# G1OJS/PyFT8

Hardware: NVIDIA B200
Metric: decoded 15-s FT8 cycles/sec (higher is better)
Workload: dtype f32

## Files before the change

pyft8_b200/csrc/fine_tc.cuh:

```cuda
#pragma once
#include <cuda_runtime.h>
#include <stdint.h>
#include "fine.cuh"

namespace ft8 {

struct TScanOut { int32_t tt; float score0; };

constexpr int FS_WIN = 224;
constexpr int FS_CAND = 32;
constexpr int FS_K1 = 64, FS_NU = 328, FS_K = FS_K1 + FS_NU, FS_KC = 8, FS_CHUNKS = FS_K / FS_KC;
constexpr int FS_N = 64;
constexpr int FS_TILES = 4;
constexpr int FS_STAGES = 4;
constexpr int FS_ACC_COLS = FS_TILES * FS_N;
constexpr int FS_A_STAGE_COLS = FS_TILES * 16;
constexpr int FS_B_SPLIT_BYTES = 2 * FS_N * 16;
constexpr int FS_B_STAGE_BYTES = 2 * FS_B_SPLIT_BYTES;
constexpr int FS_GEN_WARPS = 16;
constexpr int FS_BSTAGES = 8;
constexpr int FS_ISSUERS = 4;
constexpr int FS_NT = (FS_GEN_WARPS + FS_ISSUERS + 1) * 32;
constexpr int FS_W_LEN = 6400;
constexpr int FS_SMEM_BYTES = FS_BSTAGES * FS_B_STAGE_BYTES + FS_W_LEN * 8;
constexpr int FS_BMAT_FLOATS = FS_CHUNKS * FS_B_STAGE_BYTES / 4;
static_assert(FS_ACC_COLS + FS_STAGES * FS_A_STAGE_COLS == 512, "TMEM column plan");

__host__ __device__ __forceinline__ int fs_u_of(int j) { return j < 164 ? j - 182 : j + 554; }

__device__ __forceinline__ uint32_t smem_u32(const void* p) { return (uint32_t)__cvta_generic_to_shared(p); }
__device__ __forceinline__ void mbar_init(uint32_t a, int count) { asm volatile("mbarrier.init.shared::cta.b64 [%0], %1;" ::"r"(a), "r"(count)); }
__device__ __forceinline__ void mbar_expect_tx(uint32_t a, int bytes) {
    asm volatile("mbarrier.arrive.expect_tx.shared::cta.b64 _, [%0], %1;" ::"r"(a), "r"(bytes) : "memory");
}
__device__ __forceinline__ void mbar_wait(uint32_t a, uint32_t parity) {
    uint32_t done = 0;
    for (uint32_t spin = 0; !done; ++spin) {
        asm volatile("{\n\t.reg .pred p;\n\tmbarrier.try_wait.parity.shared::cta.b64 p, [%1], %2;\n\tselp.u32 %0, 1, 0, p;\n\t}"
                     : "=r"(done) : "r"(a), "r"(parity) : "memory");
        if (spin > (1u << 24)) __trap();
    }
}
__device__ __forceinline__ void bulk_g2s(uint32_t dst, const void* src, int bytes, uint32_t mbar) {
    asm volatile("cp.async.bulk.shared::cluster.global.mbarrier::complete_tx::bytes [%0], [%1], %2, [%3];"
                 ::"r"(dst), "l"(src), "r"(bytes), "r"(mbar) : "memory");
}
__device__ __forceinline__ void fence_proxy_async() { asm volatile("fence.proxy.async.shared::cta;" ::: "memory"); }
__device__ __forceinline__ void tc_fence_before() { asm volatile("tcgen05.fence::before_thread_sync;" ::: "memory"); }
__device__ __forceinline__ void tc_fence_after() { asm volatile("tcgen05.fence::after_thread_sync;" ::: "memory"); }
__device__ __forceinline__ void tc_commit(uint32_t mbar) {
    asm volatile("tcgen05.commit.cta_group::1.mbarrier::arrive::one.shared::cluster.b64 [%0];" ::"r"(mbar) : "memory");
}
__device__ __forceinline__ uint64_t umma_desc(uint32_t saddr, int lbo_bytes, int sbo_bytes) {
    return (uint64_t)((saddr >> 4) & 0x3FFF) | ((uint64_t)((lbo_bytes >> 4) & 0x3FFF) << 16) | ((uint64_t)((sbo_bytes >> 4) & 0x3FFF) << 32) |
           (1ull << 46);
}
constexpr uint32_t FS_IDESC = (1u << 4) | (2u << 7) | (2u << 10) | ((FS_N >> 3) << 17) | ((128u >> 4) << 24);
__device__ __forceinline__ void umma_tf32(uint32_t d_tmem, uint64_t da, uint64_t db, uint32_t accumulate) {
    asm volatile("{\n\t.reg .pred p;\n\tsetp.ne.b32 p, %4, 0;\n\t"
                 "tcgen05.mma.cta_group::1.kind::tf32 [%0], %1, %2, %3, {%5, %5, %5, %5}, p;\n\t}"
                 ::"r"(d_tmem), "l"(da), "l"(db), "r"(FS_IDESC), "r"(accumulate), "r"(0u) : "memory");
}
__device__ __forceinline__ void tmem_ld32(uint32_t taddr, uint32_t (&v)[32]) {
    asm volatile("tcgen05.ld.sync.aligned.32x32b.x32.b32 "
                 "{%0, %1, %2, %3, %4, %5, %6, %7, %8, %9, %10, %11, %12, %13, %14, %15, "
                 "%16, %17, %18, %19, %20, %21, %22, %23, %24, %25, %26, %27, %28, %29, %30, %31}, [%32];"
                 : "=r"(v[0]), "=r"(v[1]), "=r"(v[2]), "=r"(v[3]), "=r"(v[4]), "=r"(v[5]), "=r"(v[6]), "=r"(v[7]), "=r"(v[8]), "=r"(v[9]),
                   "=r"(v[10]), "=r"(v[11]), "=r"(v[12]), "=r"(v[13]), "=r"(v[14]), "=r"(v[15]), "=r"(v[16]), "=r"(v[17]), "=r"(v[18]),
                   "=r"(v[19]), "=r"(v[20]), "=r"(v[21]), "=r"(v[22]), "=r"(v[23]), "=r"(v[24]), "=r"(v[25]), "=r"(v[26]), "=r"(v[27]),
                   "=r"(v[28]), "=r"(v[29]), "=r"(v[30]), "=r"(v[31])
                 : "r"(taddr) : "memory");
}
__device__ __forceinline__ void tmem_ld_wait() { asm volatile("tcgen05.wait::ld.sync.aligned;" ::: "memory"); }
__device__ __forceinline__ float4 ldg_v4_pinned(const void* p) {
    float4 v;
    asm volatile("ld.global.nc.v4.f32 {%0, %1, %2, %3}, [%4];" : "=f"(v.x), "=f"(v.y), "=f"(v.z), "=f"(v.w) : "l"(p));
    return v;
}
__device__ __forceinline__ float2 ldg_v2_pinned(const void* p) {
    float2 v;
    asm volatile("ld.global.nc.v2.f32 {%0, %1}, [%2];" : "=f"(v.x), "=f"(v.y) : "l"(p));
    return v;
}
__device__ __forceinline__ float tf32_hi(float x) { return __uint_as_float(__float_as_uint(x) & 0xFFFFE000u); }

__device__ __forceinline__ void fine_pass12_split_finish(const FineIn& in, float2* dst, int tid, const float2* __restrict__ TF,
                                                         const float* taper, const float2 (&w)[8]) {
    const int p2 = tid & 127;
    float2 ax[4] = {in.ax[0], in.ax[1], in.ax[2], in.ax[3]};
    if (p2 >= 110) ax[0] = cscale(taper[p2 - 110], ax[0]);
    if (p2 < 82) ax[1] = cscale(taper[p2 + 18], ax[1]);
    if (p2 >= 106) ax[2] = cscale(taper[p2 - 106], ax[2]);
    if (p2 < 78) ax[3] = cscale(taper[p2 + 22], ax[3]);
    if (tid < 128) {
        fine_pass12_col<0>(in, ax, dst, p2, TF, w);
        fine_pass12_col<1>(in, ax, dst, p2, TF, w);
        fine_pass12_col<2>(in, ax, dst, p2, TF, w);
    } else {
        fine_pass12_col<3>(in, ax, dst, p2, TF, w);
        fine_pass12_col<4>(in, ax, dst, p2, TF, w);
    }
}

template <int NT>
__device__ __forceinline__ void fine_pass3_nt(const float2* src, float2* dst, int tid, const float2 (&tw8)[7]) {
    const int p = tid & 15;
#pragma unroll
    for (int r = 0; r < (25 * 16 + NT - 1) / NT; ++r) {
        const int q = (tid >> 4) + (NT / 16) * r;
        if (q < 25) {
            float2 a[8];
#pragma unroll
            for (int j = 0; j < 8; ++j) a[j] = src[q + 25 * p + 400 * j];
            Dft<8, true>::run(a);
            float2* d = dst + q + 201 * p;
            d[0] = a[0];
#pragma unroll
            for (int k = 1; k < 8; ++k) d[25 * k] = cmulc(a[k], tw8[k - 1]);
        }
    }
    __syncthreads();
}

template <int NT>
__device__ __forceinline__ void fine_last_full_nt(const float2* src, float2* dst, int tid) {
#pragma unroll
    for (int t0 = 0; t0 < 200; t0 += NT) {
        const int t = t0 + tid;
        if (t < 200) {
            float2 a[16];
#pragma unroll
            for (int j = 0; j < 16; ++j) a[j] = src[t + 201 * j];
            Dft<16, true>::run(a);
#pragma unroll
            for (int k = 0; k < 16; ++k) dst[t + 200 * k] = a[k];
        }
    }
    __syncthreads();
}

template <int NT>
__device__ __forceinline__ void fine_pass12_finish_nt(const FineIn& in, float2* dst, int tid, const float2* __restrict__ TF,
                                                      const float* taper, const float2 (&w)[8]) {
    if (NT == 256) fine_pass12_split_finish(in, dst, tid, TF, taper, w);
    else fine_pass12_finish(in, dst, tid, TF, taper, w);
}

struct FineItem { int slot, f0, h0, cyc, tt, ff; };

#ifndef FT_NT
#define FT_NT 128
#endif
#ifndef FT_CTAS
#define FT_CTAS (FT_NT == 128 ? 4 : 2)
#endif
#ifndef FF_CTAS
#define FF_CTAS (FT_NT == 128 ? 3 : 2)
#endif
constexpr int FT_SMEM_BYTES = (FINE_N + FINE_NP) * (int)sizeof(float2) + (16 + 100) * (int)sizeof(float) + (32 + 16 + 256) * (int)sizeof(float2);

template <int NT, int CTAS>
__global__ void __launch_bounds__(NT, CTAS)
k_fine_tscan(const float2* __restrict__ spec, int spec_stride, const int32_t* __restrict__ list, const int32_t* __restrict__ count,
             int n_direct, const int32_t* __restrict__ cycle_of, const int16_t* __restrict__ cand_f0, const int16_t* __restrict__ cand_h0,
             const float2* __restrict__ TF, TScanOut* __restrict__ tso, float2* __restrict__ zwin_out) {
    extern __shared__ float2 fine_smem[];
    float2 *px = fine_smem, *po = fine_smem + FINE_N;
    float* score = reinterpret_cast<float*>(fine_smem + FINE_N + FINE_NP);
    float* taper = score + 16;
    float2* w32 = reinterpret_cast<float2*>(taper + 100);
    float2* w16 = w32 + 32;
    float2* zwin = w16 + 16;
    const int tid = threadIdx.x, lane = tid & 31, warp = tid >> 5;
    if (tid < 32) w32[tid] = c_fine.w32[tid];
    if (tid < 16) { const float2 w = c_fine.w32[2 * tid]; w16[tid] = make_float2(w.x, -w.y); }
    if (tid < 100) taper[tid] = c_fine.taper[tid];
    __syncthreads();
    float2 tw[8];
#pragma unroll
    for (int t = 0; t < 8; ++t) tw[t] = w32[(t * (lane & 7)) & 31];
    float2 tw5[8];
#pragma unroll
    for (int k = 1; k < 5; ++k) tw5[k - 1] = __ldg(&TF[FINE_T5_OFF + (k - 1) * 128 + (tid & 127)]);
    float2 tw8[7];
#pragma unroll
    for (int k = 1; k < 8; ++k) tw8[k - 1] = __ldg(&TF[FINE_T8_OFF + (k - 1) * 16 + (tid & 15)]);
    const int n_items = list ? *count : n_direct;
    FineItem cur{}, nxt{};
    FineIn in;
    int item = blockIdx.x;
    if (item < n_items) {
        cur.slot = list ? list[item] : item;
        cur.f0 = cand_f0[cur.slot]; cur.h0 = cand_h0[cur.slot]; cur.cyc = cycle_of[cur.slot];
        fine_pass12_load(in, spec + (size_t)cur.cyc * spec_stride, 50 * cur.f0, tid & 127);
    }
    for (; item < n_items; item += gridDim.x) {
        const int h0 = cur.h0;
        const int tb0 = (h0 >= 0) ? 8 * h0 : 8 * h0 + 1;
        const int nitem = item + gridDim.x;
        const bool nhave = nitem < n_items;
        if (nhave) nxt.slot = list ? list[nitem] : nitem;
        fine_pass12_finish_nt<NT>(in, px, tid, TF, taper, tw5);
        __syncthreads();
        fine_pass3_nt<NT>(px, po, tid, tw8);
        if (nhave) { nxt.f0 = cand_f0[nxt.slot]; nxt.h0 = cand_h0[nxt.slot]; nxt.cyc = cycle_of[nxt.slot]; }
        {
            const int n0 = tb0 - 8 + 1152;
            for (int o = tid; o < 238; o += NT) {
                const int n = n0 + o;
                const int kk = n / 200, q = n - 200 * kk;
                const int r = kk & 3;
                const float sg = (r & 1) ? -1.0f : 1.0f;
                const float2 ir = make_float2(r == 0 ? 1.0f : (r == 2 ? -1.0f : 0.0f), r == 1 ? 1.0f : (r == 3 ? -1.0f : 0.0f));
                float2 y[4];
#pragma unroll
                for (int b = 0; b < 4; ++b) {
                    const float2 x0 = po[q + 201 * b], x1 = po[q + 201 * (4 + b)], x2 = po[q + 201 * (8 + b)], x3 = po[q + 201 * (12 + b)];
                    const float2 s = caxpy(sg, x2, x0), t = caxpy(sg, x3, x1);
                    y[b] = cmac(s, t, ir);
                }
                float2 acc = y[0];
#pragma unroll
                for (int b = 1; b < 4; ++b) acc = cmac(acc, y[b], w16[(b * kk) & 15]);
                zwin[o] = acc;
            }
        }
        __syncthreads();
        if (nhave) fine_pass12_load(in, spec + (size_t)nxt.cyc * spec_stride, 50 * nxt.f0, tid & 127);
        for (int st = warp; st < 8; st += NT / 32) {
            const float sc = costas_rows4(zwin, 2 * st, 0, lane, tw) + costas_rows4(zwin, 2 * st, 4, lane, tw);
            if (lane == 0) score[st] = sc;
        }
        __syncthreads();
        int tt = -8;
        float bestf = score[0];
        for (int ti = 1; ti < 8; ++ti) if (score[ti] > bestf) { bestf = score[ti]; tt = -8 + 2 * ti; }
        if (tid == 0) { TScanOut o; o.tt = tt; o.score0 = bestf; tso[item] = o; }
        for (int i = tid; i < FS_WIN; i += NT) zwin_out[(size_t)item * FS_WIN + i] = zwin[tt + 8 + i];
        __syncthreads();
        cur = nxt;
    }
}

#ifndef FS_AMB_TOL
#define FS_AMB_TOL 1e-4f
#endif
#ifndef FS_WAIT_FIRST
#define FS_WAIT_FIRST 1
#endif

struct FsCand { int spec_off; int m0; int valid; float score0; };

#ifdef FS_PROFILE
__device__ unsigned long long g_fs_prof[16];
#define FSP_T(v) const long long v = clock64()
#define FSP_ADD(i, d) do { if (lane == 0) atomicAdd(&g_fs_prof[i], (unsigned long long)(d)); } while (0)
#else
#define FSP_T(v)
#define FSP_ADD(i, d)
#endif

__device__ __forceinline__ void mbar_arrive(uint32_t a) { asm volatile("mbarrier.arrive.shared::cta.b64 _, [%0];" ::"r"(a) : "memory"); }
__device__ __forceinline__ void umma_tf32_ts(uint32_t d_tmem, uint32_t a_tmem, uint64_t db, uint32_t accumulate) {
    asm volatile("{\n\t.reg .pred p;\n\tsetp.ne.b32 p, %4, 0;\n\t"
                 "tcgen05.mma.cta_group::1.kind::tf32 [%0], [%1], %2, %3, {%5, %5, %5, %5}, p;\n\t}"
                 ::"r"(d_tmem), "r"(a_tmem), "l"(db), "r"(FS_IDESC), "r"(accumulate), "r"(0u) : "memory");
}
__device__ __forceinline__ void tmem_st4(uint32_t taddr, float a, float b, float c, float d) {
    asm volatile("tcgen05.st.sync.aligned.32x32b.x4.b32 [%0], {%1, %2, %3, %4};"
                 ::"r"(taddr), "r"(__float_as_uint(a)), "r"(__float_as_uint(b)), "r"(__float_as_uint(c)), "r"(__float_as_uint(d)) : "memory");
}
__device__ __forceinline__ void tmem_st8(uint32_t taddr, const float (&v)[8]) {
    asm volatile("tcgen05.st.sync.aligned.32x32b.x8.b32 [%0], {%1, %2, %3, %4, %5, %6, %7, %8};"
                 ::"r"(taddr), "r"(__float_as_uint(v[0])), "r"(__float_as_uint(v[1])), "r"(__float_as_uint(v[2])), "r"(__float_as_uint(v[3])),
                   "r"(__float_as_uint(v[4])), "r"(__float_as_uint(v[5])), "r"(__float_as_uint(v[6])), "r"(__float_as_uint(v[7])) : "memory");
}
__device__ __forceinline__ void tmem_st_wait() { asm volatile("tcgen05.wait::st.sync.aligned;" ::: "memory"); }

__global__ void __launch_bounds__(FS_NT, 1)
k_fscan_mma(const float2* __restrict__ spec, int spec_stride, const int32_t* __restrict__ list, const int32_t* __restrict__ count,
            int n_direct, const int32_t* __restrict__ cycle_of, const int16_t* __restrict__ cand_f0, const int16_t* __restrict__ cand_h0,
            const TScanOut* __restrict__ tso, const float2* __restrict__ zwin, const float* __restrict__ bmat,
            const float2* __restrict__ w6400, int32_t* __restrict__ ff_out, int32_t* __restrict__ amb_list,
            int32_t* __restrict__ amb_count) {
    extern __shared__ __align__(1024) unsigned char fs_smem[];
    unsigned char* bstage = fs_smem;
    float2* W = reinterpret_cast<float2*>(fs_smem + FS_BSTAGES * FS_B_STAGE_BYTES);
    __shared__ uint64_t bars[2 * FS_STAGES + 2 * FS_BSTAGES + 2];
    __shared__ uint32_t tmem_slot;
    __shared__ FsCand s_cand[2][FS_CAND];
    __shared__ float s_score[FS_CAND][8];
    const int tid = threadIdx.x, lane = tid & 31, warp = tid >> 5;
    const uint32_t bar_a = smem_u32(&bars[0]), bar_free = smem_u32(&bars[FS_STAGES]), bar_b = smem_u32(&bars[2 * FS_STAGES]);
    const uint32_t bar_bfree = smem_u32(&bars[2 * FS_STAGES + FS_BSTAGES]);
    const uint32_t bar_acc = smem_u32(&bars[2 * FS_STAGES + 2 * FS_BSTAGES]), bar_accfree = bar_acc + 8;
    for (int i = tid; i < FS_W_LEN; i += FS_NT) W[i] = __ldg(&w6400[i]);
    if (tid == 0) {
        for (int s = 0; s < FS_STAGES; ++s) { mbar_init(bar_a + 8 * s, 4); mbar_init(bar_free + 8 * s, FS_ISSUERS); }
        for (int s = 0; s < FS_BSTAGES; ++s) { mbar_init(bar_b + 8 * s, 1); mbar_init(bar_bfree + 8 * s, FS_ISSUERS); }
        mbar_init(bar_acc, FS_ISSUERS); mbar_init(bar_accfree, FS_GEN_WARPS);
        asm volatile("fence.mbarrier_init.release.cluster;" ::: "memory");
    }
    if (warp == 0) {
        asm volatile("tcgen05.alloc.cta_group::1.sync.aligned.shared::cta.b32 [%0], 512;" ::"r"(smem_u32(&tmem_slot)) : "memory");
        asm volatile("tcgen05.relinquish_alloc_permit.cta_group::1.sync.aligned;" ::: "memory");
    }
    tc_fence_before();
    __syncthreads();
    tc_fence_after();
    const uint32_t tmem_base = tmem_slot;
    const int n_items = list ? *count : n_direct;
    const int n_pass = (n_items + FS_CAND - 1) / FS_CAND;
    const int my_passes = (int)blockIdx.x < n_pass ? (n_pass - 1 - (int)blockIdx.x) / (int)gridDim.x + 1 : 0;

    if (warp == FS_GEN_WARPS + FS_ISSUERS) {
        if (lane == 0) {
            const uint32_t total = (uint32_t)my_passes * FS_CHUNKS;
            for (uint32_t j = 0; j < total; ++j) {
                const uint32_t bs = j % FS_BSTAGES, use = j / FS_BSTAGES;
                if (use >= 1) mbar_wait(bar_bfree + 8 * bs, (use - 1) & 1);
                mbar_expect_tx(bar_b + 8 * bs, FS_B_STAGE_BYTES);
                bulk_g2s(smem_u32(bstage + bs * FS_B_STAGE_BYTES), bmat + (size_t)(j % FS_CHUNKS) * (FS_B_STAGE_BYTES / 4), FS_B_STAGE_BYTES,
                         bar_b + 8 * bs);
            }
        }
    } else if (warp >= FS_GEN_WARPS) {
        if (lane == 0) {
            const int t = warp - FS_GEN_WARPS;
            const uint32_t total = (uint32_t)my_passes * FS_CHUNKS;
            const uint32_t d = tmem_base + t * FS_N;
            const uint64_t db0 = umma_desc(smem_u32(bstage), FS_N * 16, 128);
            for (uint32_t it = 0; it < total; ++it) {
                FSP_T(i0);
                const uint32_t st = it % FS_STAGES, use = it / FS_STAGES, c = it % FS_CHUNKS, pass_no = it / FS_CHUNKS;
                const uint32_t bs = it % FS_BSTAGES, buse = it / FS_BSTAGES;
                FSP_T(i1);
                if (c == 0 && pass_no >= 1) mbar_wait(bar_accfree, (pass_no - 1) & 1);
                FSP_T(i2);
                mbar_wait(bar_a + 8 * st, use & 1);
                FSP_T(i3);
                mbar_wait(bar_b + 8 * bs, buse & 1);
                FSP_T(i4);
                if (t == 0) { FSP_ADD(0, i1 - i0); FSP_ADD(1, i2 - i1); FSP_ADD(2, i3 - i2); FSP_ADD(3, i4 - i3); FSP_ADD(5, 1); }
                tc_fence_after();
                const uint64_t db_hi = db0 + (uint64_t)(bs * (FS_B_STAGE_BYTES >> 4)), db_lo = db_hi + (FS_B_SPLIT_BYTES >> 4);
                const uint32_t a_hi = tmem_base + FS_ACC_COLS + st * FS_A_STAGE_COLS + 16 * t;
                umma_tf32_ts(d, a_hi, db_hi, c > 0);
#ifndef FS_DEBUG_ONE_PRODUCT
                umma_tf32_ts(d, a_hi + 8, db_hi, 1);
                umma_tf32_ts(d, a_hi, db_lo, 1);
#endif
                tc_commit(bar_free + 8 * st);
                tc_commit(bar_bfree + 8 * bs);
                if (c == FS_CHUNKS - 1) tc_commit(bar_acc);
                FSP_T(i5);
                if (t == 0) FSP_ADD(4, i5 - i4);
            }
        }
    } else {
        const int gw = warp, grp = gw >> 2, s_sym = lane & 7;
        const int cl0 = 4 * (gw & 3) + (lane >> 3);
        const uint32_t lane_field = (uint32_t)(32 * (gw & 3)) << 16;
        const bool vec_ok = (spec_stride & 1) == 0;
        for (int pn = 0; pn < my_passes; ++pn) {
            const int pass = blockIdx.x + pn * gridDim.x;
            FsCand* sc_buf = s_cand[pn & 1];
            if (tid < FS_CAND) {
                const int item = pass * FS_CAND + tid;
                FsCand c; c.valid = item < n_items; c.spec_off = 0; c.m0 = 0; c.score0 = 0.f;
                if (c.valid) {
                    const int slot = list ? list[item] : item;
                    const int h0 = cand_h0[slot];
                    const int tb0 = (h0 >= 0) ? 8 * h0 : 8 * h0 + 1;
                    const TScanOut t = tso[item];
                    c.spec_off = cycle_of[slot] * spec_stride + 50 * (int)cand_f0[slot];
                    c.m0 = (2 * (tb0 + t.tt + 1152) + 31) % FS_W_LEN;
                    c.score0 = t.score0;
                }
                sc_buf[tid] = c;
            }
            asm volatile("bar.sync 1, %0;" ::"n"(FS_GEN_WARPS * 32) : "memory");
            bool ok[2]; int m[2]; const float* zrow[2]; const float2* srow[2]; float2 rot[2];
#pragma unroll
            for (int rr = 0; rr < 2; ++rr) {
                const FsCand cd = sc_buf[cl0 + 16 * rr];
                ok[rr] = cd.valid && s_sym < 7;
                m[rr] = (cd.m0 + 64 * s_sym) % FS_W_LEN;
                zrow[rr] = reinterpret_cast<const float*>(zwin) + ((size_t)(pass * FS_CAND + cl0 + 16 * rr) * FS_WIN + 32 * s_sym) * 2;
                srow[rr] = spec + cd.spec_off;
                rot[rr] = W[m[rr]];
            }
            float2 cur[2][8], nxt[2][8];
            auto load_chunk = [&](int c, float2 (&d)[2][8]) {
#pragma unroll
                for (int rr = 0; rr < 2; ++rr) {
                    if (!ok[rr]) continue;
                    if (c < FS_K1 / FS_KC) {
                        const float4 a = ldg_v4_pinned(zrow[rr] + 8 * c);
                        const float4 b = ldg_v4_pinned(zrow[rr] + 8 * c + 4);
                        d[rr][0] = make_float2(a.x, a.y); d[rr][1] = make_float2(a.z, a.w);
                        d[rr][2] = make_float2(b.x, b.y); d[rr][3] = make_float2(b.z, b.w);
                    } else {
                        const int j0 = (c - FS_K1 / FS_KC) * FS_KC;
#pragma unroll
                        for (int q = 0; q < 2; ++q) {
                            const float2* p = srow[rr] + fs_u_of(j0 + 4 * q);
                            if (vec_ok) {
                                const float4 a = ldg_v4_pinned(p), b = ldg_v4_pinned(p + 2);
                                d[rr][4 * q] = make_float2(a.x, a.y); d[rr][4 * q + 1] = make_float2(a.z, a.w);
                                d[rr][4 * q + 2] = make_float2(b.x, b.y); d[rr][4 * q + 3] = make_float2(b.z, b.w);
                            } else {
#pragma unroll
                                for (int e = 0; e < 4; ++e) d[rr][4 * q + e] = ldg_v2_pinned(p + e);
                            }
                        }
                    }
                }
            };
            load_chunk(grp, cur);
            FSP_T(p0);
            for (int c = grp; c < FS_CHUNKS; c += 4) {
                FSP_T(g0);
                if (c + 4 < FS_CHUNKS) load_chunk(c + 4, nxt);
                const uint32_t it = (uint32_t)pn * FS_CHUNKS + c, st = it % FS_STAGES, use = it / FS_STAGES;
#if FS_WAIT_FIRST
                if (use >= 1) mbar_wait(bar_free + 8 * st, (use - 1) & 1);
                tc_fence_after();
                const uint32_t ta = tmem_base + lane_field + FS_ACC_COLS + st * FS_A_STAGE_COLS;
#pragma unroll
                for (int rr = 0; rr < 2; ++rr) {
                    float re[8], im[8];
                    if (!ok[rr]) {
#pragma unroll
                        for (int e = 0; e < 8; ++e) { re[e] = 0.f; im[e] = 0.f; }
                    } else if (c < FS_K1 / FS_KC) {
#pragma unroll
                        for (int e = 0; e < 4; ++e) {
                            const float2 z = cur[rr][e];
                            re[2 * e] = z.x; re[2 * e + 1] = -z.y;
                            im[2 * e] = z.y; im[2 * e + 1] = z.x;
                        }
                    } else {
                        const int j0 = (c - FS_K1 / FS_KC) * FS_KC;
#pragma unroll
                        for (int q = 0; q < 2; ++q) {
                            float2 ph = W[((fs_u_of(j0 + 4 * q) + FS_W_LEN) * m[rr]) % FS_W_LEN];
#pragma unroll
                            for (int e = 0; e < 4; ++e) {
                                const float2 a = cur[rr][4 * q + e];
                                re[4 * q + e] = fmaf(a.x, ph.x, -a.y * ph.y);
                                im[4 * q + e] = fmaf(a.x, ph.y, a.y * ph.x);
                                if (e < 3) ph = make_float2(fmaf(ph.x, rot[rr].x, -ph.y * rot[rr].y), fmaf(ph.x, rot[rr].y, ph.y * rot[rr].x));
                            }
                        }
                    }
                    float hi[8], lo[8];
#pragma unroll
                    for (int e = 0; e < 8; ++e) { hi[e] = tf32_hi(re[e]); lo[e] = re[e] - hi[e]; }
                    tmem_st8(ta + 32 * rr, hi);
                    tmem_st8(ta + 32 * rr + 8, lo);
#pragma unroll
                    for (int e = 0; e < 8; ++e) { hi[e] = tf32_hi(im[e]); lo[e] = im[e] - hi[e]; }
                    tmem_st8(ta + 32 * rr + 16, hi);
                    tmem_st8(ta + 32 * rr + 24, lo);
                }
#else
                float re[2][8], im[2][8];
#pragma unroll
                for (int rr = 0; rr < 2; ++rr) {
                    if (!ok[rr]) {
#pragma unroll
                        for (int e = 0; e < 8; ++e) { re[rr][e] = 0.f; im[rr][e] = 0.f; }
                    } else if (c < FS_K1 / FS_KC) {
#pragma unroll
                        for (int e = 0; e < 4; ++e) {
                            const float2 z = cur[rr][e];
                            re[rr][2 * e] = z.x; re[rr][2 * e + 1] = -z.y;
                            im[rr][2 * e] = z.y; im[rr][2 * e + 1] = z.x;
                        }
                    } else {
                        const int j0 = (c - FS_K1 / FS_KC) * FS_KC;
#pragma unroll
                        for (int q = 0; q < 2; ++q) {
                            float2 ph = W[((fs_u_of(j0 + 4 * q) + FS_W_LEN) * m[rr]) % FS_W_LEN];
#pragma unroll
                            for (int e = 0; e < 4; ++e) {
                                const float2 a = cur[rr][4 * q + e];
                                re[rr][4 * q + e] = fmaf(a.x, ph.x, -a.y * ph.y);
                                im[rr][4 * q + e] = fmaf(a.x, ph.y, a.y * ph.x);
                                if (e < 3) ph = make_float2(fmaf(ph.x, rot[rr].x, -ph.y * rot[rr].y), fmaf(ph.x, rot[rr].y, ph.y * rot[rr].x));
                            }
                        }
                    }
                }
                FSP_T(g1);
                if (use >= 1) mbar_wait(bar_free + 8 * st, (use - 1) & 1);
                FSP_T(g2);
                tc_fence_after();
                const uint32_t ta = tmem_base + lane_field + FS_ACC_COLS + st * FS_A_STAGE_COLS;
#pragma unroll
                for (int rr = 0; rr < 2; ++rr) {
                    float hi[8], lo[8];
#pragma unroll
                    for (int e = 0; e < 8; ++e) { hi[e] = tf32_hi(re[rr][e]); lo[e] = re[rr][e] - hi[e]; }
                    tmem_st8(ta + 32 * rr, hi);
                    tmem_st8(ta + 32 * rr + 8, lo);
#pragma unroll
                    for (int e = 0; e < 8; ++e) { hi[e] = tf32_hi(im[rr][e]); lo[e] = im[rr][e] - hi[e]; }
                    tmem_st8(ta + 32 * rr + 16, hi);
                    tmem_st8(ta + 32 * rr + 24, lo);
                }
#endif
                tmem_st_wait();
                tc_fence_before();
                __syncwarp();
                if (lane == 0) mbar_arrive(bar_a + 8 * st);
                FSP_T(g3);
                if (gw == 0) { FSP_ADD(6, g1 - g0); FSP_ADD(7, g2 - g1); FSP_ADD(8, g3 - g2); FSP_ADD(9, 1); }
#pragma unroll
                for (int rr = 0; rr < 2; ++rr)
#pragma unroll
                    for (int e = 0; e < 8; ++e) cur[rr][e] = nxt[rr][e];
            }
            FSP_T(e0);
            mbar_wait(bar_acc, pn & 1);
            FSP_T(e1);
            if (gw == 0) { FSP_ADD(10, e0 - p0); FSP_ADD(11, e1 - e0); FSP_ADD(12, 1); }
            tc_fence_after();
            {
                const int epair = (gw >> 2) & 1, fh = gw >> 3;
                uint32_t vr[32], vi[32];
                tmem_ld32(tmem_base + lane_field + (2 * epair) * FS_N + 32 * fh, vr);
                tmem_ld32(tmem_base + lane_field + (2 * epair + 1) * FS_N + 32 * fh, vi);
                tmem_ld_wait();
                tc_fence_before();
                __syncwarp();
                if (lane == 0) mbar_arrive(bar_accfree);
                const int costas_t = (0x2560413 >> (4 * min(lane & 7, 6))) & 7;
                float sc[4];
#pragma unroll
                for (int f = 0; f < 4; ++f) {
                    float a = 0.f;
#pragma unroll
                    for (int t = 0; t < 7; ++t) {
                        const float x = __uint_as_float(vr[8 * f + t]), y = __uint_as_float(vi[8 * f + t]);
                        const float gmag = sqrtf(fmaf(x, x, y * y)) * (1.0f / 3200.0f);
                        a += (t == costas_t) ? gmag : gmag * (-1.0f / 6.0f);
                    }
                    a = ((lane & 7) < 7) ? a : 0.f;
                    a += __shfl_xor_sync(0xffffffffu, a, 1);
                    a += __shfl_xor_sync(0xffffffffu, a, 2);
                    a += __shfl_xor_sync(0xffffffffu, a, 4);
                    sc[f] = a;
                }
                if ((lane & 7) == 0) {
                    const int ecl = 16 * epair + 4 * (gw & 3) + (lane >> 3);
#pragma unroll
                    for (int f = 0; f < 4; ++f) s_score[ecl][4 * fh + f] = sc[f];
                }
            }
            asm volatile("bar.sync 1, %0;" ::"n"(FS_GEN_WARPS * 32) : "memory");
            if (tid < FS_CAND && sc_buf[tid].valid) {
                float bestf = sc_buf[tid].score0;
                int best_fi = 4;
                float second = -INFINITY, scale = fabsf(bestf);
#pragma unroll
                for (int e = 0; e < 8; ++e) {
                    const int fi = e < 4 ? e : e + 1;
                    const float v = s_score[tid][e];
                    scale = fmaxf(scale, fabsf(v));
                    if (v > bestf || (v == bestf && fi < best_fi)) { second = bestf; bestf = v; best_fi = fi; }
                    else second = fmaxf(second, v);
                }
                ff_out[pass * FS_CAND + tid] = -32 + 8 * best_fi;
                if (amb_list && bestf - second <= FS_AMB_TOL * scale) {
                    const int item = pass * FS_CAND + tid;
                    amb_list[atomicAdd(amb_count, 1)] = list ? list[item] : item;
                }
            }
        }
    }
    tc_fence_before();
    __syncthreads();
    if (warp == 0) asm volatile("tcgen05.dealloc.cta_group::1.sync.aligned.b32 %0, 512;" ::"r"(tmem_base) : "memory");
}

#ifndef FF_EARLY_LOAD
#define FF_EARLY_LOAD 1
#endif
constexpr int FF_SMEM_BYTES = (FINE_N + FINE_NP) * (int)sizeof(float2) + 100 * (int)sizeof(float) + 32 * (int)sizeof(float2);

template <int NT, int CTAS>
__global__ void __launch_bounds__(NT, CTAS)
k_fine_final(const float2* __restrict__ spec, int spec_stride, const int32_t* __restrict__ list, const int32_t* __restrict__ count,
             int n_direct, const int32_t* __restrict__ cycle_of, const int16_t* __restrict__ cand_f0, const int16_t* __restrict__ cand_h0,
             const float2* __restrict__ TF, const TScanOut* __restrict__ tso, const int32_t* __restrict__ ff_in,
             FineOut* __restrict__ fo, float* __restrict__ llr_fine, float* __restrict__ sig_grid) {
    extern __shared__ float2 fine_smem[];
    float2 *px = fine_smem, *po = fine_smem + FINE_N;
    float* G = reinterpret_cast<float*>(po);
    float* P = G + 79 * 8;
    float* taper = reinterpret_cast<float*>(fine_smem + FINE_N + FINE_NP);
    float2* w32 = reinterpret_cast<float2*>(taper + 100);
    const int tid = threadIdx.x, lane = tid & 31, warp = tid >> 5;
    if (tid < 32) w32[tid] = c_fine.w32[tid];
    if (tid < 100) taper[tid] = c_fine.taper[tid];
    __syncthreads();
    float2 tw[8];
#pragma unroll
    for (int t = 0; t < 8; ++t) tw[t] = w32[(t * (lane & 7)) & 31];
    float2 tw5[8];
#pragma unroll
    for (int k = 1; k < 5; ++k) tw5[k - 1] = __ldg(&TF[FINE_T5_OFF + (k - 1) * 128 + (tid & 127)]);
    float2 tw8[7];
#pragma unroll
    for (int k = 1; k < 8; ++k) tw8[k - 1] = __ldg(&TF[FINE_T8_OFF + (k - 1) * 16 + (tid & 15)]);
    const int n_items = list ? *count : n_direct;
    __shared__ int s_nsync;
    FineItem cur{}, nxt{};
    FineIn in;
    int item = blockIdx.x;
    if (item < n_items) {
        cur.slot = list ? list[item] : item;
        cur.f0 = cand_f0[cur.slot]; cur.h0 = cand_h0[cur.slot]; cur.cyc = cycle_of[cur.slot];
        cur.tt = tso[item].tt; cur.ff = ff_in[item];
        fine_pass12_load(in, spec + (size_t)cur.cyc * spec_stride, 50 * cur.f0 + cur.ff, tid & 127);
    }
    for (; item < n_items; item += gridDim.x) {
        const int slot = cur.slot, h0 = cur.h0, tt = cur.tt, ff = cur.ff;
        const int tb0 = (h0 >= 0) ? 8 * h0 : 8 * h0 + 1;
        const int nitem = item + gridDim.x;
        const bool nhave = nitem < n_items;
        if (nhave) { nxt.slot = list ? list[nitem] : nitem; nxt.tt = tso[nitem].tt; nxt.ff = ff_in[nitem]; }
        fine_pass12_finish_nt<NT>(in, px, tid, TF, taper, tw5);
        __syncthreads();
        fine_pass3_nt<NT>(px, po, tid, tw8);
        if (nhave) { nxt.f0 = cand_f0[nxt.slot]; nxt.h0 = cand_h0[nxt.slot]; nxt.cyc = cycle_of[nxt.slot]; }
        fine_last_full_nt<NT>(po, px, tid);
#if FF_EARLY_LOAD == 1
        if (nhave) fine_pass12_load(in, spec + (size_t)nxt.cyc * spec_stride, 50 * nxt.f0 + nxt.ff, tid & 127);
#endif
        for (int gi = warp; gi < 6; gi += NT / 32) {
            const int i = 4 * gi + (lane >> 3), ii = min(i, 20);
            const int row = 36 * (ii / 7) + ii % 7;
            const float g = dft32x4_mag(px, clip_start(tb0 + tt + 32 * row), lane, tw);
            if (i < 21) G[row * 8 + (lane & 7)] = g;
        }
        __syncthreads();
        if (warp == 0) {
            int hit = 0;
            if (lane < 21) {
                const int blk = lane / 7, k = lane - 7 * blk;
                const int row = 36 * blk + k;
                int am = 0;
                float mv = G[row * 8];
                for (int t = 1; t < 8; ++t) if (G[row * 8 + t] > mv) { mv = G[row * 8 + t]; am = t; }
                hit = (am == ((0x2560413 >> (4 * k)) & 7)) ? 1 : 0;
            }
            const int ns = __reduce_add_sync(0xffffffffu, hit);
            if (lane == 0) s_nsync = ns;
        }
        __syncthreads();
        const int nsync = s_nsync;
        const bool full = sig_grid != nullptr || nsync > 6;
        if (full) {
            for (int gi = warp; gi < 15; gi += NT / 32) {
                const int r = 4 * gi + (lane >> 3), rr = min(r, 57);
                const int sym = rr < 29 ? rr + 7 : rr + 14;
                const float g = dft32x4_mag(px, clip_start(tb0 + tt + 32 * sym), lane, tw);
                if (r < 58) { G[sym * 8 + (lane & 7)] = g; P[r * 8 + (lane & 7)] = 20.0f * log10f(g); }
            }
        }
#if FF_EARLY_LOAD == 0
        if (nhave) fine_pass12_load(in, spec + (size_t)nxt.cyc * spec_stride, 50 * nxt.f0 + nxt.ff, tid & 127);
#endif
        __syncthreads();
        if (sig_grid) for (int i = tid; i < 79 * 8; i += NT) sig_grid[(size_t)slot * 632 + i] = G[i];
        if (warp == 0) {
            if (full) {
                float p[2][8];
                if (lane < 29) {
#pragma unroll
                    for (int q = 0; q < 2; ++q)
#pragma unroll
                        for (int t = 0; t < 8; ++t) p[q][t] = P[(lane + 29 * q) * 8 + t];
                }
                float sd; int snr;
                llr_from_payload_warp(p, lane, llr_fine + (size_t)slot * 174, sd, snr);
                if (lane == 0) { FineOut o; o.tt = tt; o.ff = ff; o.nsync = nsync; o.sd = sd; o.snr = snr; fo[slot] = o; }
            } else if (lane == 0) {
                FineOut o; o.tt = tt; o.ff = ff; o.nsync = nsync; o.sd = 0.0f; o.snr = 0; fo[slot] = o;
            }
        }
        __syncthreads();
        cur = nxt;
    }
}

}
```

Measured before the change: 71030.

## Recur phase twiddles across chunks, drop smem W table, prefetch candidates

Replaces per-chunk table lookups of the phase twiddle with a complex recurrence carried across chunks in shared memory (s_ph, with a 32-step rotation factor), reloading from the global W table only at segment boundaries. This removes the 51 KB shared-memory copy of the twiddle table and its per-block load. Separately, the loop is split into a non-edge phase and a twiddle phase via a compile-time flag, so the per-chunk branch disappears. Candidate metadata for the next pass is filled by the last generator warp during the current pass with triple buffering, removing a barrier. The next-chunk load now issues after the TMEM store, using a single register buffer instead of cur/nxt. The recurrence risks accumulated rounding error, and the remaining twiddle lookups now go to global memory.

```diff
diff --git a/pyft8_b200/csrc/fine_tc.cuh b/pyft8_b200/csrc/fine_tc.cuh
--- a/pyft8_b200/csrc/fine_tc.cuh
+++ b/pyft8_b200/csrc/fine_tc.cuh
@@ -1,6 +1,7 @@
 #pragma once
 #include <cuda_runtime.h>
 #include <stdint.h>
+#include <type_traits>
 #include "fine.cuh"
 
 namespace ft8 {
@@ -22,7 +23,10 @@
 constexpr int FS_ISSUERS = 4;
 constexpr int FS_NT = (FS_GEN_WARPS + FS_ISSUERS + 1) * 32;
 constexpr int FS_W_LEN = 6400;
-constexpr int FS_SMEM_BYTES = FS_BSTAGES * FS_B_STAGE_BYTES + FS_W_LEN * 8;
+#ifndef FS_PHASE_REC
+#define FS_PHASE_REC 1
+#endif
+constexpr int FS_SMEM_BYTES = FS_BSTAGES * FS_B_STAGE_BYTES + (FS_PHASE_REC ? 0 : FS_W_LEN * 8);
 constexpr int FS_BMAT_FLOATS = FS_CHUNKS * FS_B_STAGE_BYTES / 4;
 static_assert(FS_ACC_COLS + FS_STAGES * FS_A_STAGE_COLS == 512, "TMEM column plan");
 
@@ -245,9 +249,6 @@
 #ifndef FS_AMB_TOL
 #define FS_AMB_TOL 1e-4f
 #endif
-#ifndef FS_WAIT_FIRST
-#define FS_WAIT_FIRST 1
-#endif
 
 struct FsCand { int spec_off; int m0; int valid; float score0; };
 
@@ -285,16 +286,24 @@
             int32_t* __restrict__ amb_count) {
     extern __shared__ __align__(1024) unsigned char fs_smem[];
     unsigned char* bstage = fs_smem;
+#if FS_PHASE_REC
+    const float2* __restrict__ W = w6400;
+#else
     float2* W = reinterpret_cast<float2*>(fs_smem + FS_BSTAGES * FS_B_STAGE_BYTES);
+    for (int i = threadIdx.x; i < FS_W_LEN; i += FS_NT) W[i] = __ldg(&w6400[i]);
+#endif
     __shared__ uint64_t bars[2 * FS_STAGES + 2 * FS_BSTAGES + 2];
     __shared__ uint32_t tmem_slot;
-    __shared__ FsCand s_cand[2][FS_CAND];
+    __shared__ FsCand s_cand[3][FS_CAND];
     __shared__ float s_score[FS_CAND][8];
+    __shared__ float4 s_rot[2][FS_GEN_WARPS * 32];
+#if FS_PHASE_REC
+    __shared__ float4 s_ph[2][FS_GEN_WARPS * 32];
+#endif
     const int tid = threadIdx.x, lane = tid & 31, warp = tid >> 5;
     const uint32_t bar_a = smem_u32(&bars[0]), bar_free = smem_u32(&bars[FS_STAGES]), bar_b = smem_u32(&bars[2 * FS_STAGES]);
     const uint32_t bar_bfree = smem_u32(&bars[2 * FS_STAGES + FS_BSTAGES]);
     const uint32_t bar_acc = smem_u32(&bars[2 * FS_STAGES + 2 * FS_BSTAGES]), bar_accfree = bar_acc + 8;
-    for (int i = tid; i < FS_W_LEN; i += FS_NT) W[i] = __ldg(&w6400[i]);
     if (tid == 0) {
         for (int s = 0; s < FS_STAGES; ++s) { mbar_init(bar_a + 8 * s, 4); mbar_init(bar_free + 8 * s, FS_ISSUERS); }
         for (int s = 0; s < FS_BSTAGES; ++s) { mbar_init(bar_b + 8 * s, 1); mbar_init(bar_bfree + 8 * s, FS_ISSUERS); }
@@ -362,135 +371,113 @@
         const int cl0 = 4 * (gw & 3) + (lane >> 3);
         const uint32_t lane_field = (uint32_t)(32 * (gw & 3)) << 16;
         const bool vec_ok = (spec_stride & 1) == 0;
+        auto fill_cand = [&](int pass, FsCand* buf, int l) {
+            const int item = pass * FS_CAND + l;
+            FsCand c; c.valid = item < n_items; c.spec_off = 0; c.m0 = 0; c.score0 = 0.f;
+            if (c.valid) {
+                const int slot = list ? list[item] : item;
+                const int h0 = cand_h0[slot];
+                const int tb0 = (h0 >= 0) ? 8 * h0 : 8 * h0 + 1;
+                const TScanOut t = tso[item];
+                c.spec_off = cycle_of[slot] * spec_stride + 50 * (int)cand_f0[slot];
+                c.m0 = (2 * (tb0 + t.tt + 1152) + 31) % FS_W_LEN;
+                c.score0 = t.score0;
+            }
+            buf[l] = c;
+        };
         for (int pn = 0; pn < my_passes; ++pn) {
             const int pass = blockIdx.x + pn * gridDim.x;
-            FsCand* sc_buf = s_cand[pn & 1];
-            if (tid < FS_CAND) {
-                const int item = pass * FS_CAND + tid;
-                FsCand c; c.valid = item < n_items; c.spec_off = 0; c.m0 = 0; c.score0 = 0.f;
-                if (c.valid) {
-                    const int slot = list ? list[item] : item;
-                    const int h0 = cand_h0[slot];
-                    const int tb0 = (h0 >= 0) ? 8 * h0 : 8 * h0 + 1;
-                    const TScanOut t = tso[item];
-                    c.spec_off = cycle_of[slot] * spec_stride + 50 * (int)cand_f0[slot];
-                    c.m0 = (2 * (tb0 + t.tt + 1152) + 31) % FS_W_LEN;
-                    c.score0 = t.score0;
-                }
-                sc_buf[tid] = c;
-            }
-            asm volatile("bar.sync 1, %0;" ::"n"(FS_GEN_WARPS * 32) : "memory");
-            bool ok[2]; int m[2]; const float* zrow[2]; const float2* srow[2]; float2 rot[2];
+            FsCand* sc_buf = s_cand[pn % 3];
+            if (pn == 0) {
+                fill_cand(pass, s_cand[0], tid);
+                asm volatile("bar.sync 1, %0;" ::"n"(FS_GEN_WARPS * 32) : "memory");
+            }
+            bool ok[2]; int zoff[2], soff[2];
 #pragma unroll
             for (int rr = 0; rr < 2; ++rr) {
                 const FsCand cd = sc_buf[cl0 + 16 * rr];
                 ok[rr] = cd.valid && s_sym < 7;
-                m[rr] = (cd.m0 + 64 * s_sym) % FS_W_LEN;
-                zrow[rr] = reinterpret_cast<const float*>(zwin) + ((size_t)(pass * FS_CAND + cl0 + 16 * rr) * FS_WIN + 32 * s_sym) * 2;
-                srow[rr] = spec + cd.spec_off;
-                rot[rr] = W[m[rr]];
-            }
-            float2 cur[2][8], nxt[2][8];
-            auto load_chunk = [&](int c, float2 (&d)[2][8]) {
+                const int m = (cd.m0 + 64 * s_sym) % FS_W_LEN;
+                zoff[rr] = ((pass * FS_CAND + cl0 + 16 * rr) * FS_WIN + 32 * s_sym) / 2;
+                soff[rr] = cd.spec_off;
+                const float2 r1 = W[m], r32 = W[(32 * m) % FS_W_LEN];
+                s_rot[rr][tid] = make_float4(r1.x, r1.y, r32.x, r32.y);
+            }
+            auto step_of = [&](int rr) { return (sc_buf[cl0 + 16 * rr].m0 + 64 * s_sym) % FS_W_LEN; };
+            float2 v[2][8];
+#pragma unroll
+            for (int rr = 0; rr < 2; ++rr)
+#pragma unroll
+                for (int e = 0; e < 8; ++e) v[rr][e] = make_float2(0.f, 0.f);
+            auto load_chunk = [&](int c) {
 #pragma unroll
                 for (int rr = 0; rr < 2; ++rr) {
                     if (!ok[rr]) continue;
                     if (c < FS_K1 / FS_KC) {
-                        const float4 a = ldg_v4_pinned(zrow[rr] + 8 * c);
-                        const float4 b = ldg_v4_pinned(zrow[rr] + 8 * c + 4);
-                        d[rr][0] = make_float2(a.x, a.y); d[rr][1] = make_float2(a.z, a.w);
-                        d[rr][2] = make_float2(b.x, b.y); d[rr][3] = make_float2(b.z, b.w);
+                        const float4* zp = reinterpret_cast<const float4*>(zwin) + zoff[rr] + 2 * c;
+                        const float4 a = ldg_v4_pinned(zp), b = ldg_v4_pinned(zp + 1);
+                        v[rr][0] = make_float2(a.x, a.y); v[rr][1] = make_float2(a.z, a.w);
+                        v[rr][2] = make_float2(b.x, b.y); v[rr][3] = make_float2(b.z, b.w);
                     } else {
                         const int j0 = (c - FS_K1 / FS_KC) * FS_KC;
 #pragma unroll
                         for (int q = 0; q < 2; ++q) {
-                            const float2* p = srow[rr] + fs_u_of(j0 + 4 * q);
+                            const float2* p = spec + soff[rr] + fs_u_of(j0 + 4 * q);
                             if (vec_ok) {
                                 const float4 a = ldg_v4_pinned(p), b = ldg_v4_pinned(p + 2);
-                                d[rr][4 * q] = make_float2(a.x, a.y); d[rr][4 * q + 1] = make_float2(a.z, a.w);
-                                d[rr][4 * q + 2] = make_float2(b.x, b.y); d[rr][4 * q + 3] = make_float2(b.z, b.w);
+                                v[rr][4 * q] = make_float2(a.x, a.y); v[rr][4 * q + 1] = make_float2(a.z, a.w);
+                                v[rr][4 * q + 2] = make_float2(b.x, b.y); v[rr][4 * q + 3] = make_float2(b.z, b.w);
                             } else {
 #pragma unroll
-                                for (int e = 0; e < 4; ++e) d[rr][4 * q + e] = ldg_v2_pinned(p + e);
+                                for (int e = 0; e < 4; ++e) v[rr][4 * q + e] = ldg_v2_pinned(p + e);
                             }
                         }
                     }
                 }
             };
-            load_chunk(grp, cur);
+            load_chunk(grp);
             FSP_T(p0);
-            for (int c = grp; c < FS_CHUNKS; c += 4) {
+            auto chunk = [&](int c, auto edge_t) {
+                constexpr bool EDGE = decltype(edge_t)::value;
                 FSP_T(g0);
-                if (c + 4 < FS_CHUNKS) load_chunk(c + 4, nxt);
                 const uint32_t it = (uint32_t)pn * FS_CHUNKS + c, st = it % FS_STAGES, use = it / FS_STAGES;
-#if FS_WAIT_FIRST
-                if (use >= 1) mbar_wait(bar_free + 8 * st, (use - 1) & 1);
-                tc_fence_after();
-                const uint32_t ta = tmem_base + lane_field + FS_ACC_COLS + st * FS_A_STAGE_COLS;
 #pragma unroll
                 for (int rr = 0; rr < 2; ++rr) {
-                    float re[8], im[8];
-                    if (!ok[rr]) {
-#pragma unroll
-                        for (int e = 0; e < 8; ++e) { re[e] = 0.f; im[e] = 0.f; }
-                    } else if (c < FS_K1 / FS_KC) {
-#pragma unroll
-                        for (int e = 0; e < 4; ++e) {
-                            const float2 z = cur[rr][e];
-                            re[2 * e] = z.x; re[2 * e + 1] = -z.y;
-                            im[2 * e] = z.y; im[2 * e + 1] = z.x;
+                    if constexpr (!EDGE) {
+#pragma unroll
+                        for (int e = 3; e >= 0; --e) {
+                            const float2 z = v[rr][e];
+                            v[rr][2 * e] = z;
+                            v[rr][2 * e + 1] = make_float2(-z.y, z.x);
                         }
                     } else {
                         const int j0 = (c - FS_K1 / FS_KC) * FS_KC;
+                        const float4 rw = s_rot[rr][tid];
+                        const float2 rot = make_float2(rw.x, rw.y);
+#if FS_PHASE_REC
+                        const float4 phc = s_ph[rr][tid];
+                        float2 ph[2] = {make_float2(phc.x, phc.y), make_float2(phc.z, phc.w)};
+#endif
 #pragma unroll
                         for (int q = 0; q < 2; ++q) {
-                            float2 ph = W[((fs_u_of(j0 + 4 * q) + FS_W_LEN) * m[rr]) % FS_W_LEN];
+                            const int j = j0 + 4 * q;
+#if FS_PHASE_REC
+                            float2 p;
+                            if (j < 32 || (j >= 164 && j < 196)) p = W[((fs_u_of(j) + FS_W_LEN) * step_of(rr)) % FS_W_LEN];
+                            else p = cmul(ph[q], make_float2(rw.z, rw.w));
+                            ph[q] = p;
+#else
+                            float2 p = W[((fs_u_of(j) + FS_W_LEN) * step_of(rr)) % FS_W_LEN];
+#endif
 #pragma unroll
                             for (int e = 0; e < 4; ++e) {
-                                const float2 a = cur[rr][4 * q + e];
-                                re[4 * q + e] = fmaf(a.x, ph.x, -a.y * ph.y);
-                                im[4 * q + e] = fmaf(a.x, ph.y, a.y * ph.x);
-                                if (e < 3) ph = make_float2(fmaf(ph.x, rot[rr].x, -ph.y * rot[rr].y), fmaf(ph.x, rot[rr].y, ph.y * rot[rr].x));
+                                v[rr][4 * q + e] = cmul(v[rr][4 * q + e], p);
+                                if (e < 3) p = cmul(p, rot);
                             }
                         }
-                    }
-                    float hi[8], lo[8];
-#pragma unroll
-                    for (int e = 0; e < 8; ++e) { hi[e] = tf32_hi(re[e]); lo[e] = re[e] - hi[e]; }
-                    tmem_st8(ta + 32 * rr, hi);
-                    tmem_st8(ta + 32 * rr + 8, lo);
-#pragma unroll
-                    for (int e = 0; e < 8; ++e) { hi[e] = tf32_hi(im[e]); lo[e] = im[e] - hi[e]; }
-                    tmem_st8(ta + 32 * rr + 16, hi);
-                    tmem_st8(ta + 32 * rr + 24, lo);
-                }
-#else
-                float re[2][8], im[2][8];
-#pragma unroll
-                for (int rr = 0; rr < 2; ++rr) {
-                    if (!ok[rr]) {
-#pragma unroll
-                        for (int e = 0; e < 8; ++e) { re[rr][e] = 0.f; im[rr][e] = 0.f; }
-                    } else if (c < FS_K1 / FS_KC) {
-#pragma unroll
-                        for (int e = 0; e < 4; ++e) {
-                            const float2 z = cur[rr][e];
-                            re[rr][2 * e] = z.x; re[rr][2 * e + 1] = -z.y;
-                            im[rr][2 * e] = z.y; im[rr][2 * e + 1] = z.x;
-                        }
-                    } else {
-                        const int j0 = (c - FS_K1 / FS_KC) * FS_KC;
-#pragma unroll
-                        for (int q = 0; q < 2; ++q) {
-                            float2 ph = W[((fs_u_of(j0 + 4 * q) + FS_W_LEN) * m[rr]) % FS_W_LEN];
-#pragma unroll
-                            for (int e = 0; e < 4; ++e) {
-                                const float2 a = cur[rr][4 * q + e];
-                                re[rr][4 * q + e] = fmaf(a.x, ph.x, -a.y * ph.y);
-                                im[rr][4 * q + e] = fmaf(a.x, ph.y, a.y * ph.x);
-                                if (e < 3) ph = make_float2(fmaf(ph.x, rot[rr].x, -ph.y * rot[rr].y), fmaf(ph.x, rot[rr].y, ph.y * rot[rr].x));
-                            }
-                        }
+#if FS_PHASE_REC
+                        s_ph[rr][tid] = make_float4(ph[0].x, ph[0].y, ph[1].x, ph[1].y);
+#endif
                     }
                 }
                 FSP_T(g1);
@@ -500,28 +487,31 @@
                 const uint32_t ta = tmem_base + lane_field + FS_ACC_COLS + st * FS_A_STAGE_COLS;
 #pragma unroll
                 for (int rr = 0; rr < 2; ++rr) {
-                    float hi[8], lo[8];
-#pragma unroll
-                    for (int e = 0; e < 8; ++e) { hi[e] = tf32_hi(re[rr][e]); lo[e] = re[rr][e] - hi[e]; }
-                    tmem_st8(ta + 32 * rr, hi);
-                    tmem_st8(ta + 32 * rr + 8, lo);
-#pragma unroll
-                    for (int e = 0; e < 8; ++e) { hi[e] = tf32_hi(im[rr][e]); lo[e] = im[rr][e] - hi[e]; }
-                    tmem_st8(ta + 32 * rr + 16, hi);
-                    tmem_st8(ta + 32 * rr + 24, lo);
-                }
-#endif
+#pragma unroll
+                    for (int h = 0; h < 2; ++h) {
+                        float hre[4], lre[4], him[4], lim[4];
+#pragma unroll
+                        for (int e = 0; e < 4; ++e) {
+                            const float2 x = v[rr][4 * h + e], hh = make_float2(tf32_hi(x.x), tf32_hi(x.y)), l = csub(x, hh);
+                            hre[e] = hh.x; him[e] = hh.y; lre[e] = l.x; lim[e] = l.y;
+                        }
+                        tmem_st4(ta + 32 * rr + 4 * h, hre[0], hre[1], hre[2], hre[3]);
+                        tmem_st4(ta + 32 * rr + 8 + 4 * h, lre[0], lre[1], lre[2], lre[3]);
+                        tmem_st4(ta + 32 * rr + 16 + 4 * h, him[0], him[1], him[2], him[3]);
+                        tmem_st4(ta + 32 * rr + 24 + 4 * h, lim[0], lim[1], lim[2], lim[3]);
+                    }
+                }
                 tmem_st_wait();
                 tc_fence_before();
                 __syncwarp();
                 if (lane == 0) mbar_arrive(bar_a + 8 * st);
+                if (c + 4 < FS_CHUNKS) load_chunk(c + 4);
                 FSP_T(g3);
                 if (gw == 0) { FSP_ADD(6, g1 - g0); FSP_ADD(7, g2 - g1); FSP_ADD(8, g3 - g2); FSP_ADD(9, 1); }
-#pragma unroll
-                for (int rr = 0; rr < 2; ++rr)
-#pragma unroll
-                    for (int e = 0; e < 8; ++e) cur[rr][e] = nxt[rr][e];
-            }
+            };
+            for (int c = grp; c < FS_K1 / FS_KC; c += 4) chunk(c, std::false_type{});
+            if (gw == FS_GEN_WARPS - 1 && pn + 1 < my_passes) fill_cand(pass + gridDim.x, s_cand[(pn + 1) % 3], lane);
+            for (int c = grp + FS_K1 / FS_KC; c < FS_CHUNKS; c += 4) chunk(c, std::true_type{});
             FSP_T(e0);
             mbar_wait(bar_acc, pn & 1);
             FSP_T(e1);
```

New measurement: 72290, median of 6. 1.8% higher.
